# Linux-cpp-lisp/sitator

Measured on AMD Instinct MI355X. Metric: landmark-vectors/sec (frames x mobile atoms), fill + site assignment, higher is better.
Workload: dtype f64; 1 GPU; C2: SCgrid(8,8,8) orthorhombic 32.0x35.2x38.4 A, S=D=512 (V=8), M=64, A=576 (BASELINE configs[1]), 100000 frames per GPU; frames_per_gpu=100000, n_mobile=64, n_static=512, landmark_dim=512, parallelism=frame-sharded x1

## Files before the change

### sitator_amd/_lib.py

```python
import ctypes as C
import os

import numpy as np

from . import errors

_HERE = os.path.dirname(os.path.abspath(__file__))
LIB_PATH = os.environ.get("SITATOR_LIB") or os.path.join(_HERE, "lib", "libsitator_hip.so")

OK, E_INVALID, E_HIP, E_STATIC_THRESHOLD, E_STATIC_UNASSIGNED, E_ZERO_LANDMARK, \
    E_MULTIPLE_OCCUPANCY, E_NOT_CONVERGED, E_CAPACITY, RETRY = range(10)

_dp = C.POINTER(C.c_double)
_ip = C.POINTER(C.c_int64)
_i32p = C.POINTER(C.c_int32)
_u8p = C.POINTER(C.c_uint8)
_vp = C.c_void_p
i64 = C.c_int64


class SitError(C.Structure):
    _fields_ = [("kind", C.c_int32), ("frame", C.c_int64), ("index", C.c_int64), ("aux", C.c_int64)]


# ... 583 lines not shown
    def comm_broadcast(self, arr, root):
        assert arr.flags.c_contiguous
        self._check(self.lib.sit_comm_broadcast(self._h, arr.ctypes.data_as(C.c_void_p), arr.nbytes, int(root)))
        return arr

    def comm_barrier(self):
        self._check(self.lib.sit_comm_barrier(self._h))

    def comm_attach(self, comm_ctx):
        self._check(self.lib.sit_comm_attach(self._h, comm_ctx._h if comm_ctx is not None else None))

    def timers(self):
        t = np.zeros(8)
        self.lib.sit_timers(self._h, _d(t), 8)
        return dict(zip(["fill", "fit", "predict", "gram", "site_centers", "occupancy", "h2d"], t))

    def timer_totals(self):
        t = np.zeros(24)
        self.lib.sit_timers(self._h, _d(t), 24)
        names = ["fill", "fit", "predict", "gram", "site_centers", "occupancy", "h2d"]
        return {k: (float(t[8 + i]), int(t[16 + i])) for i, k in enumerate(names)}

    def info(self):
        v = np.zeros(28)
        self.lib.sit_info(self._h, _d(v), 28)
        keys = ["row_width", "mean_candidates_loose", "tight_width", "mean_candidates_tight", "delta",
                "fallback_frames"]
        out = dict(zip(keys, v[:6]))
        out["grid_loose"] = [int(x) for x in v[6:9]]
        out["grid_tight"] = [int(x) for x in v[9:12]]
        out["frames_per_workgroup"] = int(v[12])
        out["fit_batches"], out["fit_serial_rows"], out["fit_rewalks"] = int(v[13]), int(v[14]), int(v[15])
        out["fill_kernel"], out["survivors_per_wave"], out["waves_per_workgroup"] = int(v[16]), int(v[17]), int(v[18])
        out["fit_capacity_hit"], out["fit_stop_row"] = int(v[19]), int(v[20])
        out["task_table_per_wave"] = int(v[21])
        out["assignment_fused"] = bool(v[22])
        out["band_redos"] = int(v[23])
        out["census"] = [float(x) for x in v[24:28]]
        return out

    def synchronize(self):
        self._check(self.lib.sit_synchronize(self._h))


def _settling(fn):
    import functools

    @functools.wraps(fn)
    def wrapper(self, *args, **kwargs):
        if self._deferred:
            rc, _, err = self.fill_result()
            self._check(rc, err)
        return fn(self, *args, **kwargs)
    return wrapper


for _name in ("rows_dense", "rows_sparse", "fit_push_stored_rows", "predict", "assignments", "count_zero_rows", "gram",
              "gram_limbs", "weighted_row_sums", "weighted_row_sums_limbs", "best_match", "best_match_groups",
              "site_anchors", "site_sums", "check_occupancy", "site_counts", "jump_sources", "jump_list",
              "jump_analysis", "assign_last_known", "running_mode", "set_centers"):
    setattr(HipContext, _name, _settling(getattr(HipContext, _name)))
# ... 2 lines not shown
```

### sitator_amd/csrc/ctx.hip

```cpp
#include <cmath>
#include <cstring>
#include <cstdlib>

#include <mutex>
#include <vector>

#include <cstddef>
#include "sit_internal.h"

namespace {
struct PoolEnt { void *p; size_t bytes; int device; bool idle; unsigned long long stamp; };
std::mutex g_pool_mu;
std::vector<PoolEnt> g_pool;
unsigned long long g_pool_clock = 0;

size_t pool_env_mb(const char *name, size_t dflt)
{
    const char *v = getenv(name);
    if (!v || !*v) return dflt;
    const long long x = atoll(v);
    return x < 0 ? dflt : (size_t)x;
}
size_t pool_min_bytes() { static const size_t v = pool_env_mb("SITATOR_POOL_MIN_MB", 1) << 20; return v; }
size_t g_live = 0, g_live_peak = 0;
// ... 211 lines not shown

extern "C" const char *sit_last_message(sit_ctx *c) { return c ? c->msg.c_str() : "null context"; }

extern "C" int sit_abi(int32_t *out, int n)
{
    const int32_t v[6] = {SIT_ABI_VERSION, (int32_t)sizeof(sit_error), (int32_t)sizeof(sit_fill_params),
                          (int32_t)offsetof(sit_fill_params, predict_threshold), (int32_t)offsetof(sit_error, frame), 128};
    if (out) for (int i = 0; i < n && i < 6; i++) out[i] = v[i];
    return 6;
}

extern "C" int sit_timers(sit_ctx *c, double *ms, int n)
{
    if (!c || !ms) return SIT_ERR_INVALID;
    (void)hipSetDevice(c->device);
    for (int i = 0; i < T_N; i++) stage_timer_resolve(c, i);
    for (int i = 0; i < n; i++) ms[i] = i < T_N ? c->timers[i] : (i < 2 * T_N ? c->timer_sum[i - T_N] : (i < 3 * T_N ? c->timer_cnt[i - 2 * T_N] : 0.0));
    return SIT_OK;
}

extern "C" int sit_info(sit_ctx *c, double *out, int n)
{
    if (!c || !out) return SIT_ERR_INVALID;
    const double v[28] = {(double)c->W, c->mean_candidates, (double)c->W_tight, c->tight_mean_candidates,
                          c->tight_delta, (double)c->fallback_frames, (double)c->G[0], (double)c->G[1],
                          (double)c->G[2], (double)c->tG[0], (double)c->tG[1], (double)c->tG[2], (double)c->last_fpb,
                          (double)c->ff_batches, (double)c->ff_serial_rows, (double)c->ff_rewalks,
                          (double)c->last_kernel, (double)c->last_iw, (double)c->last_nw, (double)c->ff_why, (double)c->ff_stop_row, (double)c->last_tt, c->last_fused ? 1.0 : 0.0, (double)c->band_redos,
                          c->census[0], c->census[1], c->census[2], c->census[3]};
    for (int i = 0; i < n; i++) out[i] = i < 28 ? v[i] : 0.0;
    return SIT_OK;
}

extern "C" int sit_synchronize(sit_ctx *c)
{
    if (!c) return SIT_ERR_INVALID;
    HIP_TRY(c, hipSetDevice(c->device));
    HIP_TRY(c, hipStreamSynchronize(c->stream));
    return fill_results_landed(c);
}


__global__ void k_wrap_points(Pbc P, double *pts, i64 n)
{
    i64 i = (i64)blockIdx.x * blockDim.x + threadIdx.x;
    if (i >= n) return;
    double x = pts[3 * i], y = pts[3 * i + 1], z = pts[3 * i + 2];
    wrap3(P, x, y, z);
    pts[3 * i] = x; pts[3 * i + 1] = y; pts[3 * i + 2] = z;
}

__global__ void k_distances(Pbc P, double ax, double ay, double az, const double *pts, i64 n, double *out)
{
// ... 228 lines not shown
```

### sitator_amd/csrc/fill.hip

```cpp
#include <cmath>

#include <algorithm>
#include <atomic>
#include <chrono>
#include <cstdio>
#include <cstdlib>
#include <cstring>
#include <mutex>
#include <thread>
#include <vector>

#include "sit_internal.h"

struct FillArgs {
    Pbc P;
    const double *frames;
    const i32 *static_idx, *mobile_idx;
    const double *ref_static;
    const i32 *verts;
    const double *vcd;
    const i32 *bin_off, *bin_list;
    const i32 *lattice_map;
    i32 *row_nnz, *row_idx;
    double *row_val;
// ... 579 lines not shown
            c->rows_W = W; c->rows_N = N;
        }
        if (assign && (!c->d_labels || c->assign_N != N)) {
            if ((rc = dev_alloc(c, &c->d_labels, N))) return rc;
            if ((rc = dev_alloc(c, &c->d_confs, N))) return rc;
            c->assign_N = N;
        }
        if (v3 && c->F > 0 && (rc = ensure_tight_table(c))) return rc;
        bool pred_reset = false;
        if (!want_fuse || c->F == 0) {
            if ((rc = assign && !p->dynamic_lattice_mapping ? predict_reset_with_fill(c, &pred_reset) : reset_fill_words(c))) return rc;
        }
        if (c->F == 0) {
            if (n_all_zero) *n_all_zero = 0;
            c->rows_valid = store; c->assign_valid = assign;
            if (assign) HIP_TRY(c, hipMemsetAsync(c->d_counts, 0, sizeof(i64) * (size_t)c->K, c->stream));
            return SIT_OK;
        }
        bool fused = false;
        {
            StageTimer timer(c, T_FILL);
            if (p->dynamic_lattice_mapping && (rc = launch_lattice_map(c, p))) return rc;
            if (v3) rc = fill3_launch(c, p, store, 0, -1, want_fuse, &fused);
            else { c->last_kernel = 1; c->last_fused = false; rc = launch_fill_v1(c, p); }
            if (rc) return rc;
            timer.stop();
        }
        c->rows_valid = store || !fused;
        c->assign_valid = false;
        if (assign) {
            if (fused) rc = predict_listed_rows(c, p->predict_threshold, c->fuse_wlist, c->fuse_wcount, c->fuse_seg_cap, c->fuse_nseg);
            else rc = sit_predict_internal(c, p->predict_threshold, pred_reset);
            if (rc) return rc;
        }
        FillPending &s = ring->slot[(ring->head + ring->count) % FILL_RING];
        if (!s.ev) HIP_TRY(c, hipEventCreateWithFlags(&s.ev, hipEventDisableTiming));
        s.host = (u64 *)((char *)c->h_pinned + 512) + 9 * ((ring->head + ring->count) % FILL_RING);
        s.v3 = v3; s.rows_measured = rows_measured; s.live = true;
        s.seq = ++ring->seq;
        if (!rows_measured) ring->last_rigorous_seq = s.seq;
        HIP_TRY(c, hipMemcpyAsync(s.host, c->d_err, 72, hipMemcpyDeviceToHost, c->stream));
        HIP_TRY(c, hipEventRecord(s.ev, c->stream));
        ring->count++;
        if (p->defer) {
            if (n_all_zero) *n_all_zero = -1;
            return SIT_OK;
        }
// ... 348 lines not shown
```

### sitator_amd/csrc/fill3.hip

```cpp
#include <cmath>
#include <cstdio>
#include <cstdlib>
#include <mutex>
#include <vector>
#include <algorithm>
#include <cstring>

#include "sit_internal.h"

#define F3_EXPN 128

struct Fill3Args {
    const uint4 *vh;
    const uint4 *vh16;
    const unsigned char *nvtab;
    const uint4 *pack;
    const i32 *p_off, *f_off;
    const i32 *lattice_map;
    i32 *row_nnz, *row_idx;
    double *row_val;
    i64 N;
    int D, W;
    int pG0, pG1, pG2, fG0, fG1, fG2;
    unsigned f_base;
// ... 210 lines not shown
    }
    f0 -= floor(f0); f1 -= floor(f1); f2 -= floor(f2);
    int b0 = (int)(f0 * G0), b1 = (int)(f1 * G1), b2 = (int)(f2 * G2);
    b0 = b0 < 0 ? 0 : (b0 >= G0 ? G0 - 1 : b0);
    b1 = b1 < 0 ? 0 : (b1 >= G1 ? G1 - 1 : b1);
    b2 = b2 < 0 ? 0 : (b2 >= G2 ? G2 - 1 : b2);
    return (b0 * G1 + b1) * G2 + b2;
}

#define F3_TASK_OFFSETS(TK, R0X, R0Y, VOFF, IONOFF, STATOFF, FLX)                                                          \
    do {                                                                                                                   \
        VOFF = (R0X); STATOFF = 0u; FLX = 0u;                                                                              \
        const unsigned ion_ = (TK) & ~KMASK;                                                                               \
        if (FPB1) {                                                                                                        \
            IONOFF = ionbase + 24u * ion_;                                                                                 \
            if (DYN) VOFF = 24u * (unsigned)g.lattice_map[f0 * S + (i64)(R0Y)];                                            \
        } else {                                                                                                           \
            const uint4 ir = ((const uint4 *)ionrec)[ion_];                                                                \
            IONOFF = ir.y; STATOFF = ir.z; FLX = ir.w;                                                                     \
            if (DYN) VOFF = 24u * (unsigned)g.lattice_map[(f0 + (i64)ir.w) * S + (i64)(R0Y)];                              \
        }                                                                                                                  \
    } while (0)

#define F3_D0_PASSES(NP0)                                                                                                  \
    do {                                                                                                                   \
        uint4 en_[NP0];                                                                                                    \
        unsigned ionoff_[NP0], statoff_[NP0], tfl_[NP0];                                                                   \
        int ion_[NP0];                                                                                                     \
        unsigned long long vmask_[NP0];                                                                                    \
        _Pragma("unroll") for (int u = 0; u < NP0; u++) {                                                                  \
            const int b_ = base + 64 * u, t = b_ + lane;                                                                   \
            vmask_[u] = first_lanes(nlt0 - b_);                                                                            \
            const uint2 mw = *(const uint2 *)(mark + (b_ >> 5));                            \
            const unsigned m_lo = (unsigned)__builtin_amdgcn_readfirstlane((int)mw.x), m_hi = (unsigned)__builtin_amdgcn_readfirstlane((int)mw.y); \
            const unsigned rk = __builtin_amdgcn_mbcnt_hi(m_hi, __builtin_amdgcn_mbcnt_lo(m_lo, (unsigned)carry));         \
            carry += __builtin_popcount(m_lo) + __builtin_popcount(m_hi);                                                  \
            en_[u] = make_uint4(0u, 0u, 0u, 0x7ff00000u);           \
            statoff_[u] = 0u; tfl_[u] = 0u;                                                                                \
            if (FPB1) {                                                                                                    \
                const uint2 rr = ((const uint2 *)ionrec)[rk];                                                              \
                ion_[u] = (int)rr.y;                                                                                       \
                if (F3_LANES(vmask_[u])) en_[u] = pack[rr.x + (unsigned)t];                                                \
                ionoff_[u] = ionbase + 24u * (unsigned)ion_[u];                                                            \
            } else {                                                                                                       \
                ion_[u] = (int)rk2ion[rk];                                                                                 \
                const uint4 ir = ((const uint4 *)ionrec)[ion_[u]];                                                         \
                if (F3_LANES(vmask_[u])) en_[u] = pack[ir.x + (unsigned)t];                                                \
                ionoff_[u] = ir.y; statoff_[u] = ir.z; tfl_[u] = ir.w;                                                     \
            }                                                                                                              \
        }                                                                                                                  \
        _Pragma("unroll") for (int u = 0; u < NP0; u++) {                                                                  \
            const uint4 en = en_[u];                                                                                       \
            unsigned voff = en.y;                                                                                          \
            if (DYN) voff = 24u * (unsigned)g.lattice_map[(f0 + (i64)tfl_[u]) * S + (i64)(en.y / 24u)];                    \
            const double hk = __hiloint2double((int)en.w, (int)en.z);                                                      \
            const double *sp = lds_f64(statoff_[u] + voff);                                                                \
            const double *op = lds_f64(ionoff_[u]);                                                                        \
            double qx = sp[0] + op[0], qy = sp[1] + op[1], qz = sp[2] + op[2];                                             \
            double d2;                                                                                                     \
            if (CHEAP) {                                                                                                   \
                       \
                                                           \
                qx = minimg1(qx, P.ci[0], P.cm[0]); qy = minimg1(qy, P.ci[4], P.cm[4]); qz = minimg1(qz, P.ci[8], P.cm[8]); \
                d2 = __builtin_fma(qz, qz, __builtin_fma(qy, qy, qx * qx));                                                \
            } else {                                                                                                       \
                wrapc3<CELL>(P, qx, qy, qz);                                                                               \
                const double dx = qx - P.cen[0], dy = qy - P.cen[1], dz = qz - P.cen[2];                                   \
                d2 = (dx * dx + dy * dy) + dz * dz;                                                                        \
            }                                                                                                              \
            const unsigned long long km = __ballot(!(d2 > hk)) & vmask_[u];                                                \
            if (F3_LANES(km)) ttab[mask_rank(km, t_end)] = (en.x & KMASK) | (unsigned)ion_[u];                             \
            t_end += __popcll(km);                                                                                         \
        }                                                                                                                  \
// ... 174 lines not shown
                               g.seg_cap, lane);                                                                           \
        }                                                                                                                  \
    } while (0)

template <int N>
__device__ __forceinline__ double dpp_row_shl(double x)
{
    const int lo = __double2loint(x), hi = __double2hiint(x);
    return __hiloint2double(__builtin_amdgcn_mov_dpp(hi, 0x100 + N, 0xf, 0xf, true),
                            __builtin_amdgcn_mov_dpp(lo, 0x100 + N, 0xf, 0xf, true));
}

#define F3_STAMP(var) do { if (DBG == 2 && dbg >= 10) var = __builtin_amdgcn_s_memtime(); } while (0)
#define F3_SPAN(mode, word, t0, t1) do { if (DBG == 2 && dbg == (mode) && lane == 0) atomicAdd(&g.dbgbuf[4 * (blockIdx.x & 1023u) + (word)], (u64)((t1) - (t0))); } while (0)

#ifndef F3_WPE
#define F3_WPE 7
#endif
#if F3_WPE > 0
#define F3_WPE_ATTR __attribute__((amdgpu_waves_per_eu(NW == 16 ? 8 : F3_WPE, NW == 16 ? 8 : F3_WPE)))
#else
#define F3_WPE_ATTR
#endif
template <int CELL, int LG, int NW, int DYN, int FPB1, int DBG, int FUSE>
__global__ __launch_bounds__(NW * 64) F3_WPE_ATTR void k_fill3(Fill3Head h, Fill3ArgsPtr full)
{
    constexpr int VP = 1 << LG;
    constexpr bool CHEAP = CELL == 1;
    constexpr int NT = NW * 64;
    constexpr int TPP = 64 >> LG;
    constexpr int KSH = CELL == 1 ? LG + 4 : LG + 5;
    constexpr int RSH = KSH - LG;
    constexpr unsigned KMASK = ~((1u << KSH) - 1u);
    constexpr unsigned long long LEADS = LG == 4 ? 0x0001000100010001ull : (LG == 3 ? 0x0101010101010101ull : 0x1111111111111111ull);
    extern __shared__ __attribute__((aligned(16))) char smem[];
    const int S = h.S, M = h.M, SM = S + M;
    const int fpb = FPB1 ? 1 : h.fpb;
    const int tid = threadIdx.x, lane = tid & 63, wave = __builtin_amdgcn_readfirstlane(tid >> 6);
    const int rcap = h.rcap, IW = h.iw, TT = h.tt;
    const int dbg = DBG ? h.debug_stop : 0;
    F3Layout L;
    L.fmax = h.lay[0]; L.gsync = h.lay[1]; L.ioninfo = h.lay[2]; L.etab = h.lay[3]; L.wave0 = h.lay[4]; L.o_ionrec = h.lay[5];
    L.o_ttab = h.lay[6]; L.o_sv = h.lay[7]; L.o_nzc = h.lay[8]; L.o_mark = h.lay[9]; L.wbytes = h.lay[10]; L.total = h.lay[11];
    double *xyz = (double *)smem;
    u64 *fmax = (u64 *)(smem + L.fmax);
    unsigned *wflag = (unsigned *)(fmax + fpb);
    unsigned *garrive = (unsigned *)(smem + L.gsync);
    unsigned *wspill = garrive + NW;
    uint2 *ioninfo = (uint2 *)(smem + L.ioninfo);
// ... 6 lines not shown
    unsigned *nzc = (unsigned *)(wp + L.o_nzc);
    unsigned *mark = (unsigned *)(wp + L.o_mark);
    unsigned char *rk2ion = (unsigned char *)(wp + L.o_ionrec) + 16 * IW;
    const Pbc &P = h.P;
    const i64 f0 = h.fbeg + (i64)blockIdx.x * fpb;
    const int nf = FPB1 ? 1 : (int)((h.F - f0) < fpb ? (h.F - f0) : fpb);
    const u64 errw = (u64)(S + 1 + M);
    const Fill3Args __attribute__((address_space(4))) &g = *full;

    if ((unsigned)(size_t)(__attribute__((address_space(3))) char *)smem != 0u) {
        if (tid == 0) atomicMin(g.err, 0ull);
        return;
    }
    unsigned long long ts0 = 0, ts1 = 0, ts2 = 0, ts3 = 0, ts4 = 0, tsa = 0, tsb = 0, acc_d0 = 0, acc_d1 = 0;
    F3_STAMP(ts0);
    const int prio1 = h.prio & 3;
    if (prio1) f3_setprio(prio1);
    if (tid < fpb) fmax[tid] = 0ull;
    if (CHEAP && !DYN) for (int q = tid; q < 2 * ((fpb * S + 63) / 64); q += NT) wflag[q] = 0u;
    if (FUSE && tid < 2 * NW) garrive[tid] = 0u;
    double etv = 0.0;
    if (tid < F3_EXPN) etv = h.exptab[tid];
    for (int q = lane; q < TT; q += 64) ttab[q] = 0u;
    for (int q = lane; q < (FPB1 ? 2 * (IW + 1) : 4 * IW + (IW + 4) / 4); q += 64) ionrec[q] = 0u;
    {
        const double *fbase = h.frames + (g.frame_mod > 0 ? f0 % g.frame_mod : f0) * h.A * 3;
        if (h.contig == 4) {
            const int n2 = (nf * SM * 3 + 1) >> 1;
            const char *src = (const char *)fbase;
            for (int e0 = wave * 64; e0 < n2; e0 += NT) {
                if (e0 + lane < n2)
                    __builtin_amdgcn_global_load_lds((const __attribute__((address_space(1))) void *)(src + 16 * (size_t)(e0 + lane)),
                                                     (__attribute__((address_space(3))) void *)(smem + 16 * e0), 16, 0, 2);
            }
        } else if (h.contig == 3) {
            const int n2 = (nf * SM * 3) >> 1;
            const double2 *src2 = (const double2 *)fbase;
            double2 *dst2 = (double2 *)xyz;
            for (int e0 = tid; e0 < n2; e0 += 4 * NT) {
                double2 v[4];
#pragma unroll
                for (int u = 0; u < 4; u++) { const int e = e0 + u * NT; v[u] = e < n2 ? src2[e] : make_double2(0.0, 0.0); }
#pragma unroll
                for (int u = 0; u < 4; u++) { const int e = e0 + u * NT; if (e < n2) dst2[e] = v[u]; }
            }
        } else if (h.contig == 2) {
            const int n = nf * SM * 3;
// ... 51 lines not shown
                        need_store = true;
                        atomicOr(&wflag[(fl * S + r) >> 5], 1u << ((fl * S + r) & 31));
                    }
                    const double c0 = CHEAP ? g.cen[0] : P.cen[0], c1 = CHEAP ? g.cen[1] : P.cen[1], c2 = CHEAP ? g.cen[2] : P.cen[2];
                    double qx = x + (c0 - rx), qy = y + (c1 - ry), qz = z + (c2 - rz_);
                    wrapc3<CELL>(P, qx, qy, qz);
                    const double dx = -qx + c0, dy = -qy + c1, dz = -qz + c2;
                    const double d2 = (dx * dx + dy * dy) + dz * dz;
                    if (d2 > g.delta2) {
                        atomicOr(&fmax[fl], 1ull);
                        if (d2 > g.thr2_lo && (d2 > g.thr2_hi || sqrt(d2) > g.static_thr))
                            atomicMin(g.err, (u64)(g.frame0 + f0 + fl) * errw + (u64)r);
                    }
                }
            }
            if (need_store) { d[0] = x; d[1] = y; d[2] = z; }
        } else {
            wrapc3<CELL>(P, x, y, z);
            if (CHEAP) { d[0] = -x; d[1] = -y; d[2] = -z; }
            else { d[0] = P.cen[0] - x; d[1] = P.cen[1] - y; d[2] = P.cen[2] - z; }
            const int b = bin_of3<CELL>(P, x, y, z, g.pG0, g.pG1, g.pG2);
            i32 lo, hi;
            { uint2 pr; __builtin_memcpy(&pr, g.p_off + b, 8); lo = (i32)pr.x; hi = (i32)pr.y; }
            unsigned fb = 0u;
            if (h.has_fallback) fb = (unsigned)bin_of3<CELL>(P, x, y, z, g.fG0, g.fG1, g.fG2);
            ioninfo[fl * M + (r - S)] = make_uint2((unsigned)lo, (unsigned)(hi - lo) | (fb << 8));
        }
    }
    F3_STAMP(tsb);
    __syncthreads();
    F3_STAMP(ts2);
    F3_SPAN(10, 1, ts1, ts2); F3_SPAN(12, 2, ts1, tsb); F3_SPAN(12, 3, tsb, ts2);
    if (tid < nf && h.has_fallback) {
        const bool tight = DYN ? (g.frame_dmax[f0 + tid] * g.frame_dmax[f0 + tid] <= g.delta2) : (fmax[tid] == 0ull);
        if (!tight) atomicAdd(&g.scal[2], 1ull);
    }
    if (dbg == 1) return;
    if (prio1) __builtin_amdgcn_s_setprio(0);

    const char *vh = CHEAP ? (const char *)g.vh16 : (const char *)g.vh;
    const uint4 *pack = g.pack;
    const ExpK ek = expk_make(g.midpoint, g.steepness);
    const double x0lo = g.x0lo;
    const int nvu = g.nv_uniform;
    const int hh = lane & (VP - 1), gi = lane >> LG;
    const unsigned hh32 = (unsigned)hh << RSH;
    const unsigned long long ltmask = (1ull << lane) - 1ull;
    const unsigned xyz_s = 24u * (unsigned)S;
    const int GW = FUSE ? (IW <= 32 ? 64 / IW : 1) : 1;

    const int nions = nf * M;
    bool spilled = false;
    for (int ib0 = wave * IW; ib0 < nions; ib0 += NW * IW) {
        const int nib = (nions - ib0) < IW ? (nions - ib0) : IW;
        int fl = 0, j = 0, nL = 0;
        unsigned lo = 0u;
        if (lane < nib) {
            const int ion = ib0 + lane;
            if (!FPB1) for (int q = 1; q < nf; q++) fl += ion >= q * M;
            j = ion - fl * M;
            const uint2 ii = ioninfo[ion];
            lo = ii.x; nL = (int)(ii.y & 255u);
            if (h.has_fallback) {
                const bool tight = DYN ? (g.frame_dmax[f0 + fl] * g.frame_dmax[f0 + fl] <= g.delta2) : (fmax[fl] == 0ull);
                if (!tight) {
                    const unsigned fb = ii.y >> 8;
                    uint2 pr;
                    __builtin_memcpy(&pr, g.f_off + fb, 8);
                    nL = (int)(pr.y - pr.x); lo = g.f_base + pr.x;
                }
            }
        }
        const int inL = wave_add_scan(nL), exL = inL - nL;
        const int nlt = __builtin_amdgcn_readlane(inL, 63);
        if (nlt > h.mcap) { if (lane == 0) atomicAdd(&g.scal[3], 1ull); break; }
        for (int q = lane; q < 2 * ((nlt + 63) >> 6); q += 64) mark[q] = 0u;
        {
            const unsigned long long nem = __ballot(nL > 0);
            if (lane < nib) {
                if (nL > 0) {
                    const int rk = mask_rank(nem, 0);
                    atomicOr(&mark[(inL - 1) >> 5], 1u << ((inL - 1) & 31));
                    if (FPB1) ((uint2 *)ionrec)[rk] = make_uint2(lo - (unsigned)exL, (unsigned)lane);
                    else rk2ion[rk] = (unsigned char)lane;
                }
                if (!FPB1) ((uint4 *)ionrec)[lane] = make_uint4(lo - (unsigned)exL, 24u * (unsigned)(fl * SM + S + j), 24u * (unsigned)(fl * SM), (unsigned)fl);
                nzc[lane] = 0u;
            }
        }
        if (DBG && dbg == 9 && lane == 0) { atomicAdd(&g.scal[5], (u64)nlt); atomicAdd(&g.scal[7], 1ull); }
        const unsigned ionbase = xyz_s + 24u * (unsigned)ib0;
        F3_STAMP(ts3);
        F3_SPAN(10, 2, ts2, ts3);
        int t_end = 0, carry = 0, cnt = 0;
        spilled = false;
        const int nlt0 = (DBG && dbg == 2) ? 0 : nlt;
        for (int base = 0; base < nlt0; base += 64) {
            F3_STAMP(ts4);
            if (NW < 16 && base + 64 < nlt0 && t_end <= TT - 128) { F3_D0_PASSES(2); base += 64; }
            else F3_D0_PASSES(1);
            if (DBG == 2 && dbg >= 10) { unsigned long long tq = __builtin_amdgcn_s_memtime(); acc_d0 += tq - ts4; ts4 = tq; }
            if (t_end <= TT - 64 && base + 64 < nlt0) continue;
            if (DBG && dbg == 9 && lane == 0) atomicAdd(&g.scal[4], (u64)t_end);
            if (DBG && dbg == 3) t_end = 0;
            const int pend = (t_end + TPP - 1) / TPP;
            int cursor = 0;
            while (cursor < pend) {
                while (cursor < pend && cnt + TPP <= rcap) {
                    if (cursor + 1 < pend && cnt + 2 * TPP <= rcap) {
                        F3_D1E_PASSES(2);
                        cursor += 2;
                    } else {
                        F3_D1E_PASSES(1);
                        cursor += 1;
                    }
                }
                if (DBG && dbg == 9 && lane == 0) atomicAdd(&g.scal[6], (u64)cnt);
                if (cursor < pend) F3_T_ROUND(0);
            }
            t_end = 0;
            if (DBG == 2 && dbg >= 10) { unsigned long long tq = __builtin_amdgcn_s_memtime(); acc_d1 += tq - ts4; }
        }
        if (DBG && dbg == 5) cnt = 0;
        F3_STAMP(ts4);
        F3_T_ROUND(1);
// ... 170 lines not shown

__global__ __launch_bounds__(256) void k_pack_lists(const i32 *list, const unsigned char *crit, i64 n, int lg, int rsh, const uint4 *vh, uint4 *out, int hi)
{
    const i64 i = (i64)blockIdx.x * 256 + threadIdx.x;
    if (i >= n) return;
    const unsigned rec = ((unsigned)list[i] << lg) | (unsigned)crit[i];
    const unsigned off = rec << rsh;
    const uint4 r = vh[2 * (size_t)rec], r2 = vh[2 * (size_t)rec + 1];
    out[i] = hi ? make_uint4(off, r.x, r2.z, r2.w) : make_uint4(off, r.x, r2.x, r2.y);
}

static int fill3_pack_lists(sit_ctx *c, bool have_tight, bool cheap)
{
    if (c->d_pack && c->pack_gen == c->table_gen && c->pack_tight == (have_tight ? 1 : 0) && c->pack_cheap == (cheap ? 1 : 0)) return SIT_OK;
    i32 nt = 0, nl = 0;
    const i64 nbl = (i64)c->G[0] * c->G[1] * c->G[2], nbt = (i64)c->tG[0] * c->tG[1] * c->tG[2];
    HIP_TRY(c, hipMemcpyAsync(&nl, c->d_bin_off + nbl, 4, hipMemcpyDeviceToHost, c->stream));
    if (have_tight) HIP_TRY(c, hipMemcpyAsync(&nt, c->d_tbin_off + nbt, 4, hipMemcpyDeviceToHost, c->stream));
    HIP_TRY(c, hipStreamSynchronize(c->stream));
    SIT_REQUIRE(c, (i64)nt + (i64)nl < (1LL << 28), "sit_fill: candidate tables too large for the third-generation kernel");
    int rc;
    if ((rc = dev_alloc(c, &c->d_pack, 4 * ((i64)nt + (i64)nl + 1)))) return rc;
    uint4 *pk = (uint4 *)c->d_pack;
    const int lg = f3_vp(c) == 16 ? 4 : (f3_vp(c) == 8 ? 3 : 2), rsh = cheap ? 4 : 5;
    if (nt > 0) k_pack_lists<<<dim3((unsigned)((nt + 255) / 256)), dim3(256), 0, c->stream>>>(c->d_tbin_list, c->d_tbin_crit, nt, lg, rsh, (const uint4 *)c->d_vh, pk, cheap ? 1 : 0);
    if (nl > 0) k_pack_lists<<<dim3((unsigned)((nl + 255) / 256)), dim3(256), 0, c->stream>>>(c->d_bin_list, c->d_bin_crit, nl, lg, rsh, (const uint4 *)c->d_vh, pk + nt, cheap ? 1 : 0);
    HIP_TRY(c, hipGetLastError());
    c->pack_nt = nt; c->pack_gen = c->table_gen; c->pack_tight = have_tight ? 1 : 0; c->pack_cheap = cheap ? 1 : 0;
    return SIT_OK;
}

bool fill3_eligible(sit_ctx *c)
{
    if (c->fill_kernel != 3) return false;
    if (c->Vp > 16) return false;
    if (c->D >= (1LL << 22) || c->M > 30000 || c->W > 255) return false;
    if ((c->S + c->M) * 24 + c->M * 8 > 132 * 1024) return false;
    return true;
}

static hipError_t f3_dispatch(sit_ctx *c, const Fill3Head &h_in, Fill3ArgsPtr full, unsigned grid, size_t lds, int nw, int vp,
                              bool diag, bool dynmap, bool fuse)
{
    Fill3Head h = h_in;
    {
        const int fpb1 = (nw != 4 || h.fpb == 1) ? 1 : 0;
        const F3Layout L = f3_layout(fpb1 ? 1 : h.fpb, h.S + h.M, h.M, nw, h.rcap, h.iw, h.tt, h.mcap, fpb1);
        const int v[12] = {L.fmax, L.gsync, L.ioninfo, L.etab, L.wave0, L.o_ionrec, L.o_ttab, L.o_sv, L.o_nzc, L.o_mark, L.wbytes, L.total};
        for (int i = 0; i < 12; i++) h.lay[i] = v[i];
    }
#define F3_LAUNCH(CELL, LGV, NWV, DY, F1, DB, FU)                                                                              \
    do {                                                                                                                   \
        hipError_t e = lds_limit((const void *)k_fill3<CELL, LGV, NWV, DY, F1, DB, FU>, lds, c->device);                   \
        if (e != hipSuccess) return e;                                                                                     \
        k_fill3<CELL, LGV, NWV, DY, F1, DB, FU><<<dim3(grid), dim3(NWV * 64), lds, c->stream>>>(h, full);                  \
    } while (0)
#define F3_PICK3(CELL, LGV, NWV, F1)                                                                                           \
    do {                                                                                                                   \
        if (dynmap) F3_LAUNCH(CELL, LGV, NWV, 1, F1, 0, 0);                                                                \
        else if (h.debug_stop >= 10) F3_LAUNCH(CELL, LGV, NWV, 0, F1, 2, 0);                                                  \
        else if (h.debug_stop) F3_LAUNCH(CELL, LGV, NWV, 0, F1, 1, 0);                                                     \
        else if (fuse) F3_LAUNCH(CELL, LGV, NWV, 0, F1, 0, 1);                                                             \
        else F3_LAUNCH(CELL, LGV, NWV, 0, F1, 0, 0);                                                                       \
    } while (0)
#define F3_PICK(CELL, LGV)                                                                                                     \
    do {                                                                                                                   \
        if (nw == 16) F3_PICK3(CELL, LGV, 16, 1); else if (nw == 8) F3_PICK3(CELL, LGV, 8, 1);                             \
        else if (h.fpb == 1) F3_PICK3(CELL, LGV, 4, 1); else F3_PICK3(CELL, LGV, 4, 0);                                    \
    } while (0)
    if (diag) { if (vp == 16) F3_PICK(1, 4); else if (vp == 8) F3_PICK(1, 3); else F3_PICK(1, 2); }
    else { if (vp == 16) F3_PICK(0, 4); else if (vp == 8) F3_PICK(0, 3); else F3_PICK(0, 2); }
#undef F3_PICK
#undef F3_PICK3
#undef F3_LAUNCH
    return hipGetLastError();
}

struct F3Tuned { i64 key[8]; int rcap, tt; };
static std::mutex g_f3_mutex;
static std::vector<F3Tuned> g_f3_tuned;

#define F3_ARGS_BYTES 1024
#define F3_TRIAL_WORDS 17

int fill3_prepare(sit_ctx *c)
{
// ... 123 lines not shown
    if (rcap_auto) {
        auto wg_per_cu = [&](int r) {
            const size_t b = (lds_bytes(nw, fpb, r) + 1535) / 1024 * 1024, cap = (size_t)((nw == 16 ? 32 : 28) / nw);
            const size_t k = (160 * 1024) / b;
            return k > cap ? cap : k;
        };
        for (int r : {40, 32}) if (r >= 64 / vp && wg_per_cu(r) > wg_per_cu(rcap)) rcap = r;
    }
    if (tt_auto) {
        const double per_ion = (have_tight ? c->tight_mean_candidates : c->mean_candidates) + 1.0;
        int want = (int)(0.5 * per_ion * iw_for(nw, fpb)) + 64;
        want = want < 128 ? 128 : (want > 512 ? 512 : (want + 63) / 64 * 64);
        auto wgs = [&](int t) { const int keep = tt; tt = t; const size_t b = (lds_bytes(nw, fpb, rcap) + 1535) / 1024 * 1024; tt = keep; return (160 * 1024) / b; };
        const size_t base = wgs(128);
        int pick = 128;
        for (int t = 192; t <= want; t += 64) if (wgs(t) == base) pick = t;
        tt = pick;
    }
    while (fpb > 1 && lds_bytes(nw, fpb, rcap) > 160 * 1024 - 512) fpb--;
    SIT_REQUIRE(c, lds_bytes(nw, fpb, rcap) <= 160 * 1024 - 256, "sit_fill: one frame's atoms do not fit in LDS");
    iw = iw_for(nw, fpb);
    SIT_REQUIRE(c, (i64)iw * wmax <= 65536, "sit_fill: candidate lists too long for the third-generation kernel");
    h.fpb = fpb; h.iw = iw; h.mcap = mcap_for(iw);
    if (fuse && (i64)fpb * M > (i64)nw * iw) fuse = false;
    if (!fuse) store = true;
    a.row_val = fuse || store ? c->d_row_val : nullptr;
    a.store = store ? 1 : 0;
    const unsigned grid_all = (unsigned)((f_hi - f_lo + fpb - 1) / fpb);
    int nseg = 0;
    i64 seg_cap = 0;
    if (fuse) {
        nseg = (int)std::min<i64>((i64)grid_all > 0 ? (i64)grid_all : 1, (i64)cu_count(c) * 4);
        seg_cap = ((i64)grid_all + nseg - 1) / nseg * ((i64)fpb * M);
        if ((rc = wide_list_carve(c, nseg, seg_cap, &a.wcount, &a.wlist))) return rc;
        a.seg_cap = seg_cap; a.nseg = nseg;
        a.col_ptr = c->d_col_ptr; a.col_k = c->d_col_k; a.col_val = c->d_col_val;
        a.labels = c->d_labels; a.confs = c->d_confs;
        a.normed = c->centers_normed; a.threshold = p->predict_threshold;
    }
    if (h.debug_stop >= 10) {
        if ((rc = ensure_scratch(c, 1024 * 4 * 8 + 64))) return rc;
        a.dbgbuf = (u64 *)c->d_scratch;
        HIP_TRY(c, hipMemsetAsync(a.dbgbuf, 0, 1024 * 4 * 8, c->stream));
    }
    if (c->fill_args_host.size() != sizeof(Fill3Args) || memcmp(c->fill_args_host.data(), &a, sizeof(Fill3Args)) != 0) {
        c->fill_args_host.assign((const char *)&a, (const char *)&a + sizeof(Fill3Args));
// ... 33 lines not shown
            const hipEvent_t e0 = ev0.e, e1 = ev1.e;
            Fill3Head ht = h;
            Fill3Args at = a;
            at.err = (u64 *)(c->d_fill_args + 2 * F3_ARGS_BYTES); at.scal = at.err + 1;
            HIP_TRY(c, hipMemsetAsync(at.err, 0, F3_TRIAL_WORDS * 8, c->stream));
            HIP_TRY(c, hipMemcpyAsync(c->d_fill_args + F3_ARGS_BYTES, &at, sizeof(Fill3Args), hipMemcpyHostToDevice, c->stream));
            const Fill3ArgsPtr full_t = (Fill3ArgsPtr)(c->d_fill_args + F3_ARGS_BYTES);
            ht.F = std::min<i64>(f_hi, f_lo + (i64)4096 * fpb);
            const unsigned gt = (unsigned)((ht.F - f_lo + fpb - 1) / fpb);
            float best = 1e30f;
            int br = rcap, bt = tt;
            const int keep_tt = tt;
            for (int q = 0; q < NC; q++) {
                bool dup = false;
                for (int q2 = 0; q2 < q; q2++) dup = dup || (cand[q2][0] == cand[q][0] && cand[q2][1] == cand[q][1]);
                if (dup) continue;
                tt = cand[q][1];
                const size_t ldq = lds_bytes(nw, fpb, cand[q][0]);
                if (ldq > 160 * 1024 - 512) continue;
                ht.rcap = cand[q][0]; ht.tt = cand[q][1];
                float tq = 1e30f;
                for (int rep = 0; rep < 5; rep++) {
                    HIP_TRY(c, hipEventRecord(e0, c->stream));
                    HIP_TRY(c, f3_dispatch(c, ht, full_t, gt, ldq, nw, vp, diag, dynmap, false));
                    HIP_TRY(c, hipEventRecord(e1, c->stream));
                    HIP_TRY(c, hipEventSynchronize(e1));
                    float ms = 0;
                    HIP_TRY(c, hipEventElapsedTime(&ms, e0, e1));
                    if (rep > 0 && ms < tq) tq = ms;
                }
                if (tq < best * (q == 0 ? 1.0f : 0.96f)) { best = tq; br = cand[q][0]; bt = cand[q][1]; }
            }
            tt = keep_tt;
            rcap = br; tt = bt;
            F3Tuned t; memcpy(t.key, key, sizeof(key)); t.rcap = rcap; t.tt = tt;
            { std::lock_guard<std::mutex> lock(g_f3_mutex); g_f3_tuned.push_back(t); }
        }
    }
    const size_t lds = lds_bytes(nw, fpb, rcap);
    SIT_REQUIRE(c, lds <= 160 * 1024 - 256, "sit_fill: one frame's atoms do not fit in LDS");
    h.rcap = rcap; h.tt = tt;
    if (f3_env_int("SITATOR_DEBUG_SHAPE", 0))
        fprintf(stderr, "k_fill3 shape: nw %d fpb %d rcap %d iw %d tt %d mcap %d, %zu bytes of LDS per workgroup\n", nw, fpb, rcap, iw, tt, h.mcap, lds);
    c->last_fpb = fpb; c->last_kernel = 3; c->last_iw = rcap; c->last_nw = nw; c->last_tt = tt;
    const unsigned grid = (unsigned)((f_hi - f_lo + fpb - 1) / fpb);
    if (fused) *fused = fuse;
    c->last_fused = fuse;
    if (fuse) {
        if ((rc = reset_step_words(c, true, a.wcount, 2 * nseg))) return rc;
        c->fuse_wlist = a.wlist; c->fuse_wcount = a.wcount; c->fuse_seg_cap = seg_cap; c->fuse_nseg = nseg;
    } else if (fuse_asked && (rc = reset_fill_words(c))) return rc;
    if (f_hi <= f_lo) return SIT_OK;
    HIP_TRY(c, f3_dispatch(c, h, full, grid, lds, nw, vp, diag, dynmap, fuse));
    if (h.debug_stop >= 10) { k_f3_spans<<<dim3(1), dim3(64), 0, c->stream>>>(a.dbgbuf, c->d_scal); HIP_TRY(c, hipGetLastError()); }
    return SIT_OK;
}
```

### sitator_amd/csrc/sit_internal.h

```cpp
#pragma once

#include <hip/hip_runtime.h>
#include <stdint.h>
#include <string>
#include <vector>

#include "sitator_hip.h"

typedef int64_t i64;
typedef int32_t i32;
typedef unsigned long long u64;

struct Pbc {
    double cm[9];
    double ci[9];
    double cen[3];
};

enum { T_FILL = 0, T_FIT = 1, T_PREDICT = 2, T_GRAM = 3, T_CENTERS = 4, T_OCC = 5, T_H2D = 6, T_N = 8 };

#define SIT_NO_ERROR_KEY 0xFFFFFFFFFFFFFFFFull

struct sit_ctx {
    int device = 0;
// ... 30 lines not shown
    bool cell_diagonal = false;
    int fill_kernel = 3;
    i64 fallback_frames = 0;
    int last_fpb = 0;
    double *d_frame_dmax = nullptr;
    unsigned *d_vh = nullptr;
    unsigned *d_vh16 = nullptr;
    double *d_ref_soa = nullptr;
    unsigned char *d_nv = nullptr;
    double *d_exptab = nullptr;
    unsigned *d_pack = nullptr;
    i64 pack_nt = 0;
    i64 table_gen = 0, pack_gen = -1;
    int pack_tight = -1, pack_cheap = -1;
    bool idx_contig = false;
    i64 idx_s0 = 0, idx_m0 = 0;
    double hmin = 0;
    int last_kernel = 0, last_iw = 0, last_nw = 0, last_tt = 0;
    int nv_uniform = 0;
    i64 band_redos = 0;
    bool f3_ref_in_cell = false;
    bool f3_cheap_ok = false;
    double f3_x0lo = 0, f3_x0hi = 0;
    bool last_fused = false;
    i32 *fuse_wlist = nullptr;
    unsigned *fuse_wcount = nullptr;
    i64 fuse_seg_cap = 0;
    int fuse_nseg = 0;
    double census[4] = {0, 0, 0, 0};

    i64 F = 0, A = 0, M = 0, frame0 = 0;
    double *d_frames = nullptr;
    bool frames_owned = false;
    i64 frames_cap_bytes = 0;
    i32 *d_static_idx = nullptr, *d_mobile_idx = nullptr;
    i32 *d_lattice_map = nullptr;
    bool map_valid = false;

    i64 N = 0, rows_W = 0, rows_N = 0;
    i32 *d_row_nnz = nullptr, *d_row_idx = nullptr;
    double *d_row_val = nullptr;
    bool rows_valid = false;
    bool rows_overflowed = false;
    double rows_mean_nnz = 0;

    i64 *d_labels = nullptr;
// ... 348 lines not shown
```

Before: 8.709 billion lvec/s.

## Add slot-mapped candidate expansion to fill3 for one-frame workgroups

Adds a SLOT template variant of k_fill3 in which each lane is mapped to a fixed (ion, candidate-slot) pair with a per-frame power-of-two slot width, replacing the mark/popcount rank-compaction and ionrec table for distributing candidate entries. The frame's maximum candidate-list length is gathered with an atomicMax during binning so the slot width is chosen per frame, with a bail-out when lists exceed 64. The aim is to drop the compaction bookkeeping and LDS traffic in the dense-pass loop. The cost is idle lanes when lists are shorter than the slot width. It is enabled by default for 4-wave, one-frame-per-workgroup shapes with short primary lists.

```diff
diff --git a/sitator_amd/_lib.py b/sitator_amd/_lib.py
--- a/sitator_amd/_lib.py
+++ b/sitator_amd/_lib.py
@@ -629,8 +629,8 @@
         return {k: (float(t[8 + i]), int(t[16 + i])) for i, k in enumerate(names)}
 
     def info(self):
-        v = np.zeros(28)
-        self.lib.sit_info(self._h, _d(v), 28)
+        v = np.zeros(29)
+        self.lib.sit_info(self._h, _d(v), 29)
         keys = ["row_width", "mean_candidates_loose", "tight_width", "mean_candidates_tight", "delta",
                 "fallback_frames"]
         out = dict(zip(keys, v[:6]))
@@ -644,6 +644,7 @@
         out["assignment_fused"] = bool(v[22])
         out["band_redos"] = int(v[23])
         out["census"] = [float(x) for x in v[24:28]]
+        out["fill_slot_width"] = int(v[28])
         return out
 
     def synchronize(self):
diff --git a/sitator_amd/csrc/ctx.hip b/sitator_amd/csrc/ctx.hip
--- a/sitator_amd/csrc/ctx.hip
+++ b/sitator_amd/csrc/ctx.hip
@@ -257,13 +257,13 @@
 extern "C" int sit_info(sit_ctx *c, double *out, int n)
 {
     if (!c || !out) return SIT_ERR_INVALID;
-    const double v[28] = {(double)c->W, c->mean_candidates, (double)c->W_tight, c->tight_mean_candidates,
+    const double v[29] = {(double)c->W, c->mean_candidates, (double)c->W_tight, c->tight_mean_candidates,
                           c->tight_delta, (double)c->fallback_frames, (double)c->G[0], (double)c->G[1],
                           (double)c->G[2], (double)c->tG[0], (double)c->tG[1], (double)c->tG[2], (double)c->last_fpb,
                           (double)c->ff_batches, (double)c->ff_serial_rows, (double)c->ff_rewalks,
                           (double)c->last_kernel, (double)c->last_iw, (double)c->last_nw, (double)c->ff_why, (double)c->ff_stop_row, (double)c->last_tt, c->last_fused ? 1.0 : 0.0, (double)c->band_redos,
-                          c->census[0], c->census[1], c->census[2], c->census[3]};
-    for (int i = 0; i < n; i++) out[i] = i < 28 ? v[i] : 0.0;
+                          c->census[0], c->census[1], c->census[2], c->census[3], (double)c->last_slot};
+    for (int i = 0; i < n; i++) out[i] = i < 29 ? v[i] : 0.0;
     return SIT_OK;
 }
 
diff --git a/sitator_amd/csrc/fill.hip b/sitator_amd/csrc/fill.hip
--- a/sitator_amd/csrc/fill.hip
+++ b/sitator_amd/csrc/fill.hip
@@ -625,7 +625,7 @@
             StageTimer timer(c, T_FILL);
             if (p->dynamic_lattice_mapping && (rc = launch_lattice_map(c, p))) return rc;
             if (v3) rc = fill3_launch(c, p, store, 0, -1, want_fuse, &fused);
-            else { c->last_kernel = 1; c->last_fused = false; rc = launch_fill_v1(c, p); }
+            else { c->last_kernel = 1; c->last_fused = false; c->last_slot = 0; rc = launch_fill_v1(c, p); }
             if (rc) return rc;
             timer.stop();
         }
diff --git a/sitator_amd/csrc/fill3.hip b/sitator_amd/csrc/fill3.hip
--- a/sitator_amd/csrc/fill3.hip
+++ b/sitator_amd/csrc/fill3.hip
@@ -256,33 +256,58 @@
         }                                                                                                                  \
     } while (0)
 
-#define F3_D0_PASSES(NP0)                                                                                                  \
-    do {                                                                                                                   \
-        uint4 en_[NP0];                                                                                                    \
-        unsigned ionoff_[NP0], statoff_[NP0], tfl_[NP0];                                                                   \
-        int ion_[NP0];                                                                                                     \
-        unsigned long long vmask_[NP0];                                                                                    \
-        _Pragma("unroll") for (int u = 0; u < NP0; u++) {                                                                  \
-            const int b_ = base + 64 * u, t = b_ + lane;                                                                   \
-            vmask_[u] = first_lanes(nlt0 - b_);                                                                            \
-            const uint2 mw = *(const uint2 *)(mark + (b_ >> 5));                            \
-            const unsigned m_lo = (unsigned)__builtin_amdgcn_readfirstlane((int)mw.x), m_hi = (unsigned)__builtin_amdgcn_readfirstlane((int)mw.y); \
-            const unsigned rk = __builtin_amdgcn_mbcnt_hi(m_hi, __builtin_amdgcn_mbcnt_lo(m_lo, (unsigned)carry));         \
-            carry += __builtin_popcount(m_lo) + __builtin_popcount(m_hi);                                                  \
-            en_[u] = make_uint4(0u, 0u, 0u, 0x7ff00000u);           \
-            statoff_[u] = 0u; tfl_[u] = 0u;                                                                                \
-            if (FPB1) {                                                                                                    \
-                const uint2 rr = ((const uint2 *)ionrec)[rk];                                                              \
-                ion_[u] = (int)rr.y;                                                                                       \
-                if (F3_LANES(vmask_[u])) en_[u] = pack[rr.x + (unsigned)t];                                                \
-                ionoff_[u] = ionbase + 24u * (unsigned)ion_[u];                                                            \
-            } else {                                                                                                       \
-                ion_[u] = (int)rk2ion[rk];                                                                                 \
-                const uint4 ir = ((const uint4 *)ionrec)[ion_[u]];                                                         \
-                if (F3_LANES(vmask_[u])) en_[u] = pack[ir.x + (unsigned)t];                                                \
-                ionoff_[u] = ir.y; statoff_[u] = ir.z; tfl_[u] = ir.w;                                                     \
-            }                                                                                                              \
-        }                                                                                                                  \
+#define F3_D0_PASSES(NP0)                                                                                                   \
+    do {                                                                                                                    \
+        uint4 en_[NP0];                                                                                                     \
+        unsigned ionoff_[NP0], statoff_[NP0], tfl_[NP0];                                                                    \
+        int ion_[NP0];                                                                                                      \
+        unsigned long long vmask_[NP0];                                                                                     \
+        uint2 ii_[NP0];                                                                                                     \
+        bool in_[NP0];                                                                                                      \
+        if (SLOT) {                                                                                                         \
+             \
+             \
+                                            \
+            _Pragma("unroll") for (int u = 0; u < NP0; u++) {                                                               \
+                ion_[u] = base + d0_step * u + s_ion;                                                                       \
+                in_[u] = ion_[u] < nib;                                                                                     \
+                ii_[u] = ioninfo[ib0 + ion_[u]];                                                                            \
+                ionoff_[u] = ionbase + 24u * (unsigned)(base + d0_step * u) + s_ioff;                                       \
+            }                                                                                                               \
+                     \
+            _Pragma("unroll") for (int u = 0; u < NP0; u++) asm volatile("" : "+v"(ii_[u].x), "+v"(ii_[u].y));              \
+        }                                                                                                                   \
+        _Pragma("unroll") for (int u = 0; u < NP0; u++) {                                                                   \
+            statoff_[u] = 0u; tfl_[u] = 0u;                                                                                 \
+            if (SLOT) {                                                                                                     \
+                 \
+                 \
+                const bool act_ = in_[u] && s_slot < (int)(ii_[u].y & 255u);                                                \
+                vmask_[u] = __ballot(act_);                                                                                 \
+                en_[u] = pack[act_ ? ii_[u].x + (unsigned)s_slot : 0u];                                                     \
+            } else {                                                                                                        \
+                en_[u] = make_uint4(0u, 0u, 0u, 0x7ff00000u);       \
+                const int b_ = base + 64 * u, t = b_ + lane;                                                                \
+                vmask_[u] = first_lanes(nlt0 - b_);                                                                         \
+                const uint2 mw = *(const uint2 *)(mark + (b_ >> 5));                        \
+                const unsigned m_lo = (unsigned)__builtin_amdgcn_readfirstlane((int)mw.x), m_hi = (unsigned)__builtin_amdgcn_readfirstlane((int)mw.y); \
+                const unsigned rk = __builtin_amdgcn_mbcnt_hi(m_hi, __builtin_amdgcn_mbcnt_lo(m_lo, (unsigned)carry));      \
+                carry += __builtin_popcount(m_lo) + __builtin_popcount(m_hi);                                               \
+                if (FPB1) {                                                                                                 \
+                    const uint2 rr = ((const uint2 *)ionrec)[rk];                                                           \
+                    ion_[u] = (int)rr.y;                                                                                    \
+                    if (F3_LANES(vmask_[u])) en_[u] = pack[rr.x + (unsigned)t];                                             \
+                    ionoff_[u] = ionbase + 24u * (unsigned)ion_[u];                                                         \
+                } else {                                                                                                    \
+                    ion_[u] = (int)rk2ion[rk];                                                                              \
+                    const uint4 ir = ((const uint4 *)ionrec)[ion_[u]];                                                      \
+                    if (F3_LANES(vmask_[u])) en_[u] = pack[ir.x + (unsigned)t];                                             \
+                    ionoff_[u] = ir.y; statoff_[u] = ir.z; tfl_[u] = ir.w;                                                  \
+                }                                                                                                           \
+            }                                                                                                               \
+        }                                                                                                                   \
+              \
+        if (SLOT) { _Pragma("unroll") for (int u = 0; u < NP0; u++) asm volatile("" : "+v"(en_[u].x)); }                    \
         _Pragma("unroll") for (int u = 0; u < NP0; u++) {                                                                  \
             const uint4 en = en_[u];                                                                                       \
             unsigned voff = en.y;                                                                                          \
@@ -503,9 +528,10 @@
 #else
 #define F3_WPE_ATTR
 #endif
-template <int CELL, int LG, int NW, int DYN, int FPB1, int DBG, int FUSE>
+template <int CELL, int LG, int NW, int DYN, int FPB1, int DBG, int FUSE, int SLOT = 0>
 __global__ __launch_bounds__(NW * 64) F3_WPE_ATTR void k_fill3(Fill3Head h, Fill3ArgsPtr full)
 {
+    static_assert(!SLOT || FPB1, "the slot form is for one frame per workgroup");
     constexpr int VP = 1 << LG;
     constexpr bool CHEAP = CELL == 1;
     constexpr int NT = NW * 64;
@@ -558,7 +584,7 @@
     double etv = 0.0;
     if (tid < F3_EXPN) etv = h.exptab[tid];
     for (int q = lane; q < TT; q += 64) ttab[q] = 0u;
-    for (int q = lane; q < (FPB1 ? 2 * (IW + 1) : 4 * IW + (IW + 4) / 4); q += 64) ionrec[q] = 0u;
+    if (!SLOT) for (int q = lane; q < (FPB1 ? 2 * (IW + 1) : 4 * IW + (IW + 4) / 4); q += 64) ionrec[q] = 0u;
     {
         const double *fbase = h.frames + (g.frame_mod > 0 ? f0 % g.frame_mod : f0) * h.A * 3;
         if (h.contig == 4) {
@@ -656,6 +682,7 @@
             const int b = bin_of3<CELL>(P, x, y, z, g.pG0, g.pG1, g.pG2);
             i32 lo, hi;
             { uint2 pr; __builtin_memcpy(&pr, g.p_off + b, 8); lo = (i32)pr.x; hi = (i32)pr.y; }
+            if (SLOT && hi - lo > 8) atomicMax((unsigned *)fmax + 2 * fl + 1, (unsigned)(hi - lo));
             unsigned fb = 0u;
             if (h.has_fallback) fb = (unsigned)bin_of3<CELL>(P, x, y, z, g.fG0, g.fG1, g.fG2);
             ioninfo[fl * M + (r - S)] = make_uint2((unsigned)lo, (unsigned)(hi - lo) | (fb << 8));
@@ -665,7 +692,17 @@
     __syncthreads();
     F3_STAMP(ts2);
     F3_SPAN(10, 1, ts1, ts2); F3_SPAN(12, 2, ts1, tsb); F3_SPAN(12, 3, tsb, ts2);
-    if (tid < nf && h.has_fallback) {
+    bool frame_tight = true;
+    int lgsl_frame = 3;
+    if (SLOT) {
+        const uint2 fm = *(const uint2 *)fmax;
+        const unsigned beyond = (unsigned)__builtin_amdgcn_readfirstlane((int)fm.x), lmax = (unsigned)__builtin_amdgcn_readfirstlane((int)fm.y);
+        if (h.has_fallback) frame_tight = DYN ? (g.frame_dmax[f0] * g.frame_dmax[f0] <= g.delta2) : beyond == 0u;
+        lgsl_frame = 3 + (lmax > 8u) + (lmax > 16u) + (lmax > 32u) + (lmax > 64u);
+    }
+    if (SLOT) {
+        if (tid == 0 && !frame_tight) atomicAdd(&g.scal[2], 1ull);
+    } else if (tid < nf && h.has_fallback) {
         const bool tight = DYN ? (g.frame_dmax[f0 + tid] * g.frame_dmax[f0 + tid] <= g.delta2) : (fmax[tid] == 0ull);
         if (!tight) atomicAdd(&g.scal[2], 1ull);
     }
@@ -689,37 +726,54 @@
         const int nib = (nions - ib0) < IW ? (nions - ib0) : IW;
         int fl = 0, j = 0, nL = 0;
         unsigned lo = 0u;
-        if (lane < nib) {
-            const int ion = ib0 + lane;
-            if (!FPB1) for (int q = 1; q < nf; q++) fl += ion >= q * M;
-            j = ion - fl * M;
-            const uint2 ii = ioninfo[ion];
-            lo = ii.x; nL = (int)(ii.y & 255u);
-            if (h.has_fallback) {
-                const bool tight = DYN ? (g.frame_dmax[f0 + fl] * g.frame_dmax[f0 + fl] <= g.delta2) : (fmax[fl] == 0ull);
-                if (!tight) {
-                    const unsigned fb = ii.y >> 8;
+        int nlt = 0, lgsl = 0;
+        if (SLOT) {
+            lgsl = lgsl_frame;
+            if (lane < nib) { j = ib0 + lane; nzc[lane] = 0u; }
+            if (h.has_fallback && !frame_tight) {
+                if (lane < nib) {
+                    const unsigned fb = ioninfo[ib0 + lane].y >> 8;
                     uint2 pr;
                     __builtin_memcpy(&pr, g.f_off + fb, 8);
-                    nL = (int)(pr.y - pr.x); lo = g.f_base + pr.x;
+                    nL = (int)(pr.y - pr.x);
+                    ioninfo[ib0 + lane] = make_uint2(g.f_base + pr.x, (unsigned)nL | (fb << 8));
+                }
+                lgsl = 3 + (__ballot(nL > 8) != 0ull) + (__ballot(nL > 16) != 0ull) + (__ballot(nL > 32) != 0ull) + (__ballot(nL > 64) != 0ull);
+            }
+            if (lgsl > 6) { if (lane == 0) atomicAdd(&g.scal[3], 1ull); break; }
+        } else {
+            if (lane < nib) {
+                const int ion = ib0 + lane;
+                if (!FPB1) for (int q = 1; q < nf; q++) fl += ion >= q * M;
+                j = ion - fl * M;
+                const uint2 ii = ioninfo[ion];
+                lo = ii.x; nL = (int)(ii.y & 255u);
+                if (h.has_fallback) {
+                    const bool tight = DYN ? (g.frame_dmax[f0 + fl] * g.frame_dmax[f0 + fl] <= g.delta2) : (fmax[fl] == 0ull);
+                    if (!tight) {
+                        const unsigned fb = ii.y >> 8;
+                        uint2 pr;
+                        __builtin_memcpy(&pr, g.f_off + fb, 8);
+                        nL = (int)(pr.y - pr.x); lo = g.f_base + pr.x;
+                    }
                 }
             }
-        }
-        const int inL = wave_add_scan(nL), exL = inL - nL;
-        const int nlt = __builtin_amdgcn_readlane(inL, 63);
-        if (nlt > h.mcap) { if (lane == 0) atomicAdd(&g.scal[3], 1ull); break; }
-        for (int q = lane; q < 2 * ((nlt + 63) >> 6); q += 64) mark[q] = 0u;
-        {
-            const unsigned long long nem = __ballot(nL > 0);
-            if (lane < nib) {
-                if (nL > 0) {
-                    const int rk = mask_rank(nem, 0);
-                    atomicOr(&mark[(inL - 1) >> 5], 1u << ((inL - 1) & 31));
-                    if (FPB1) ((uint2 *)ionrec)[rk] = make_uint2(lo - (unsigned)exL, (unsigned)lane);
-                    else rk2ion[rk] = (unsigned char)lane;
+            const int inL = wave_add_scan(nL), exL = inL - nL;
+            nlt = __builtin_amdgcn_readlane(inL, 63);
+            if (nlt > h.mcap) { if (lane == 0) atomicAdd(&g.scal[3], 1ull); break; }
+            for (int q = lane; q < 2 * ((nlt + 63) >> 6); q += 64) mark[q] = 0u;
+            {
+                const unsigned long long nem = __ballot(nL > 0);
+                if (lane < nib) {
+                    if (nL > 0) {
+                        const int rk = mask_rank(nem, 0);
+                        atomicOr(&mark[(inL - 1) >> 5], 1u << ((inL - 1) & 31));
+                        if (FPB1) ((uint2 *)ionrec)[rk] = make_uint2(lo - (unsigned)exL, (unsigned)lane);
+                        else rk2ion[rk] = (unsigned char)lane;
+                    }
+                    if (!FPB1) ((uint4 *)ionrec)[lane] = make_uint4(lo - (unsigned)exL, 24u * (unsigned)(fl * SM + S + j), 24u * (unsigned)(fl * SM), (unsigned)fl);
+                    nzc[lane] = 0u;
                 }
-                if (!FPB1) ((uint4 *)ionrec)[lane] = make_uint4(lo - (unsigned)exL, 24u * (unsigned)(fl * SM + S + j), 24u * (unsigned)(fl * SM), (unsigned)fl);
-                nzc[lane] = 0u;
             }
         }
         if (DBG && dbg == 9 && lane == 0) { atomicAdd(&g.scal[5], (u64)nlt); atomicAdd(&g.scal[7], 1ull); }
@@ -729,12 +783,15 @@
         int t_end = 0, carry = 0, cnt = 0;
         spilled = false;
         const int nlt0 = (DBG && dbg == 2) ? 0 : nlt;
-        for (int base = 0; base < nlt0; base += 64) {
+        const int d0_lim = SLOT ? ((DBG && dbg == 2) ? 0 : nib) : nlt0, d0_step = SLOT ? 64 >> lgsl : 64;
+        const int s_ion = lane >> lgsl, s_slot = lane & ((1 << lgsl) - 1);
+        const unsigned s_ioff = 24u * (unsigned)s_ion;
+        for (int base = 0; base < d0_lim; base += d0_step) {
             F3_STAMP(ts4);
-            if (NW < 16 && base + 64 < nlt0 && t_end <= TT - 128) { F3_D0_PASSES(2); base += 64; }
+            if (NW < 16 && base + d0_step < d0_lim && t_end <= TT - 128) { F3_D0_PASSES(2); base += d0_step; }
             else F3_D0_PASSES(1);
             if (DBG == 2 && dbg >= 10) { unsigned long long tq = __builtin_amdgcn_s_memtime(); acc_d0 += tq - ts4; ts4 = tq; }
-            if (t_end <= TT - 64 && base + 64 < nlt0) continue;
+            if (t_end <= TT - 64 && base + d0_step < d0_lim) continue;
             if (DBG && dbg == 9 && lane == 0) atomicAdd(&g.scal[4], (u64)t_end);
             if (DBG && dbg == 3) t_end = 0;
             const int pend = (t_end + TPP - 1) / TPP;
@@ -951,6 +1008,7 @@
     int rc;
     if ((rc = dev_alloc(c, &c->d_pack, 4 * ((i64)nt + (i64)nl + 1)))) return rc;
     uint4 *pk = (uint4 *)c->d_pack;
+    HIP_TRY(c, hipMemsetAsync(pk + (nt + nl), 0, 16, c->stream));
     const int lg = f3_vp(c) == 16 ? 4 : (f3_vp(c) == 8 ? 3 : 2), rsh = cheap ? 4 : 5;
     if (nt > 0) k_pack_lists<<<dim3((unsigned)((nt + 255) / 256)), dim3(256), 0, c->stream>>>(c->d_tbin_list, c->d_tbin_crit, nt, lg, rsh, (const uint4 *)c->d_vh, pk, cheap ? 1 : 0);
     if (nl > 0) k_pack_lists<<<dim3((unsigned)((nl + 255) / 256)), dim3(256), 0, c->stream>>>(c->d_bin_list, c->d_bin_crit, nl, lg, rsh, (const uint4 *)c->d_vh, pk + nt, cheap ? 1 : 0);
@@ -969,7 +1027,7 @@
 }
 
 static hipError_t f3_dispatch(sit_ctx *c, const Fill3Head &h_in, Fill3ArgsPtr full, unsigned grid, size_t lds, int nw, int vp,
-                              bool diag, bool dynmap, bool fuse)
+                              bool diag, bool dynmap, bool fuse, bool slot)
 {
     Fill3Head h = h_in;
     {
@@ -978,19 +1036,19 @@
         const int v[12] = {L.fmax, L.gsync, L.ioninfo, L.etab, L.wave0, L.o_ionrec, L.o_ttab, L.o_sv, L.o_nzc, L.o_mark, L.wbytes, L.total};
         for (int i = 0; i < 12; i++) h.lay[i] = v[i];
     }
-#define F3_LAUNCH(CELL, LGV, NWV, DY, F1, DB, FU)                                                                              \
+#define F3_LAUNCH(CELL, LGV, NWV, DY, F1, DB, FU, SL)                                                                          \
     do {                                                                                                                   \
-        hipError_t e = lds_limit((const void *)k_fill3<CELL, LGV, NWV, DY, F1, DB, FU>, lds, c->device);                   \
+        hipError_t e = lds_limit((const void *)k_fill3<CELL, LGV, NWV, DY, F1, DB, FU, SL>, lds, c->device);               \
         if (e != hipSuccess) return e;                                                                                     \
-        k_fill3<CELL, LGV, NWV, DY, F1, DB, FU><<<dim3(grid), dim3(NWV * 64), lds, c->stream>>>(h, full);                  \
+        k_fill3<CELL, LGV, NWV, DY, F1, DB, FU, SL><<<dim3(grid), dim3(NWV * 64), lds, c->stream>>>(h, full);              \
     } while (0)
 #define F3_PICK3(CELL, LGV, NWV, F1)                                                                                           \
     do {                                                                                                                   \
-        if (dynmap) F3_LAUNCH(CELL, LGV, NWV, 1, F1, 0, 0);                                                                \
-        else if (h.debug_stop >= 10) F3_LAUNCH(CELL, LGV, NWV, 0, F1, 2, 0);                                                  \
-        else if (h.debug_stop) F3_LAUNCH(CELL, LGV, NWV, 0, F1, 1, 0);                                                     \
-        else if (fuse) F3_LAUNCH(CELL, LGV, NWV, 0, F1, 0, 1);                                                             \
-        else F3_LAUNCH(CELL, LGV, NWV, 0, F1, 0, 0);                                                                       \
+        if (dynmap) F3_LAUNCH(CELL, LGV, NWV, 1, F1, 0, 0, 0);                                                             \
+        else if (h.debug_stop >= 10) { if (F1 && slot) F3_LAUNCH(CELL, LGV, NWV, 0, F1, 2, 0, F1); else F3_LAUNCH(CELL, LGV, NWV, 0, F1, 2, 0, 0); } \
+        else if (h.debug_stop) F3_LAUNCH(CELL, LGV, NWV, 0, F1, 1, 0, 0);                                                  \
+        else if (fuse) { if (F1 && slot) F3_LAUNCH(CELL, LGV, NWV, 0, F1, 0, 1, F1); else F3_LAUNCH(CELL, LGV, NWV, 0, F1, 0, 1, 0); } \
+        else { if (F1 && slot) F3_LAUNCH(CELL, LGV, NWV, 0, F1, 0, 0, F1); else F3_LAUNCH(CELL, LGV, NWV, 0, F1, 0, 0, 0); } \
     } while (0)
 #define F3_PICK(CELL, LGV)                                                                                                     \
     do {                                                                                                                   \
@@ -1160,6 +1218,17 @@
     iw = iw_for(nw, fpb);
     SIT_REQUIRE(c, (i64)iw * wmax <= 65536, "sit_fill: candidate lists too long for the third-generation kernel");
     h.fpb = fpb; h.iw = iw; h.mcap = mcap_for(iw);
+    bool slot = false;
+    {
+        const int dstop = p->dynamic_lattice_mapping ? 0 : f3_env_int("SITATOR_DEBUG_STOP", 0);
+        const bool possible = (nw != 4 || fpb == 1) && wmax <= 64 && !p->dynamic_lattice_mapping && (dstop == 0 || dstop >= 10);
+        const i64 wprim = have_tight ? c->W_tight : c->W;
+        const int asked = f3_env_int("SITATOR_F3_SLOT", -1);
+        slot = possible && (asked < 0 ? (nw == 4 && wprim <= 8) : asked != 0);
+        int width = 8;
+        while (width < wmax) width *= 2;
+        c->last_slot = slot ? width : 0;
+    }
     if (fuse && (i64)fpb * M > (i64)nw * iw) fuse = false;
     if (!fuse) store = true;
     a.row_val = fuse || store ? c->d_row_val : nullptr;
@@ -1239,7 +1308,7 @@
                 float tq = 1e30f;
                 for (int rep = 0; rep < 5; rep++) {
                     HIP_TRY(c, hipEventRecord(e0, c->stream));
-                    HIP_TRY(c, f3_dispatch(c, ht, full_t, gt, ldq, nw, vp, diag, dynmap, false));
+                    HIP_TRY(c, f3_dispatch(c, ht, full_t, gt, ldq, nw, vp, diag, dynmap, false, slot));
                     HIP_TRY(c, hipEventRecord(e1, c->stream));
                     HIP_TRY(c, hipEventSynchronize(e1));
                     float ms = 0;
@@ -1268,7 +1337,7 @@
         c->fuse_wlist = a.wlist; c->fuse_wcount = a.wcount; c->fuse_seg_cap = seg_cap; c->fuse_nseg = nseg;
     } else if (fuse_asked && (rc = reset_fill_words(c))) return rc;
     if (f_hi <= f_lo) return SIT_OK;
-    HIP_TRY(c, f3_dispatch(c, h, full, grid, lds, nw, vp, diag, dynmap, fuse));
+    HIP_TRY(c, f3_dispatch(c, h, full, grid, lds, nw, vp, diag, dynmap, fuse, slot));
     if (h.debug_stop >= 10) { k_f3_spans<<<dim3(1), dim3(64), 0, c->stream>>>(a.dbgbuf, c->d_scal); HIP_TRY(c, hipGetLastError()); }
     return SIT_OK;
 }
diff --git a/sitator_amd/csrc/sit_internal.h b/sitator_amd/csrc/sit_internal.h
--- a/sitator_amd/csrc/sit_internal.h
+++ b/sitator_amd/csrc/sit_internal.h
@@ -76,6 +76,7 @@
     bool f3_ref_in_cell = false;
     bool f3_cheap_ok = false;
     double f3_x0lo = 0, f3_x0hi = 0;
+    int last_slot = 0;
     bool last_fused = false;
     i32 *fuse_wlist = nullptr;
     unsigned *fuse_wcount = nullptr;
```

Measured after the change: 9.017 billion lvec/s (median of 6 runs). 1.04x the previous value.
